# Zoe187419/ATE_replication_causalML

Hardware: AMD Instinct MI355X
Metric: rows/sec for DML-ATE cross-fit, N=1e7 p=500, 1/2/4/8 MI355X; ATE/SE parity (higher is better)
Workload: dtype bf16; 1 GPU; model=DML-PLR 5-fold cross-fit, CV-LASSO nuisances (100 lambdas, inner 4-fold CV), global_batch=10000000, seq_len=500, N=10000000, p=500, folds=5, parallelism=dp1, dgp=tutorial, n_kept=10000000, layout=blocked64+bytes8

## Files before the change

### ate_replication_causalml_amd/_native.py

```python
from __future__ import annotations

import ctypes
import os
from pathlib import Path

_LIBDIR = Path(__file__).resolve().parent / "_lib"
_hip = None
_cpu = None


class NativeMissing(RuntimeError):
    pass


class NativeError(RuntimeError):

    def __init__(self, name: str, status: int, detail: str):
        self.entry, self.status = name, status
        super().__init__(f"{name} failed with status {status}: {detail}")


HIP_ERRORS = {
    1: "hipErrorInvalidValue", 2: "hipErrorOutOfMemory", 3: "hipErrorNotInitialized",
    4: "hipErrorDeinitialized", 9: "hipErrorInvalidConfiguration",
    13: "hipErrorInvalidSymbol", 17: "hipErrorInvalidDevicePointer",
    21: "hipErrorInvalidMemcpyDirection", 35: "hipErrorInsufficientDriver",
    52: "hipErrorMissingConfiguration", 53: "hipErrorPriorLaunchFailure",
    98: "hipErrorInvalidDeviceFunction", 100: "hipErrorNoDevice", 101: "hipErrorInvalidDevice",
    200: "hipErrorInvalidImage", 201: "hipErrorInvalidContext", 209: "hipErrorNoBinaryForGpu",
    218: "hipErrorInvalidKernelFile", 400: "hipErrorInvalidHandle", 500: "hipErrorNotFound",
    600: "hipErrorNotReady", 700: "hipErrorIllegalAddress", 701: "hipErrorLaunchOutOfResources",
    702: "hipErrorLaunchTimeOut", 710: "hipErrorAssert", 719: "hipErrorLaunchFailure",
    720: "hipErrorCooperativeLaunchTooLarge", 801: "hipErrorNotSupported",
    900: "hipErrorStreamCaptureUnsupported", 901: "hipErrorStreamCaptureInvalidated",
    907: "hipErrorCapturedEvent", 999: "hipErrorUnknown",
}


def describe_status(rc: int) -> str:
    if rc < 0:
        return "rejected by the entry point's own argument check (no kernel launched)"
    return f"{HIP_ERRORS.get(rc, 'hipError?')} ({rc})"


c_void_p = ctypes.c_void_p
c_int = ctypes.c_int
c_int64 = ctypes.c_int64
c_uint64 = ctypes.c_uint64
c_double = ctypes.c_double

_SIGS = {
    "ate_gram_bf16": "pliipipipipppp",
    "ate_gram_bf16_pair": "pllipippipippippiip",
    "ate_gram_bf16_pair_bits": "pllipippipippippiip",
    "ate_last_error": "pi",
    "ate_last_stale_error": "pi",
    "ate_clear_errors": "",
    "ate_debug_bad_launch": "ip",
    "ate_check_kernel_resources": "pi",
    "ate_gram_f32": "plippipipippppp",
    "ate_gram_f64": "plippipipippppp",
    "ate_gram_tile_sizes": "pppp",
    "ate_chol_solve": "pipiipdpppppp",
    "ate_chol_solve_k": "pipipidppppp",
    "ate_spd_solve_batched": "ppiippp",
    "ate_predict": "ipllppiidipp",
    "ate_irls_update": "ipllppiiiiippppipp",
    "ate_irls_check": "piidippp",
    "ate_naive": "ippplpppp",
    "ate_clip_propensity": "pplpp",
    "ate_aipw": "ppppppldpppp",
    "ate_dml_moments": "ppplppp",
    "ate_dml_finalize": "pipp",
    "ate_boot_multinomial": "ppluiipp",
    "ate_boot_poisson": "ppluiilipp",
    "ate_enet_prepare": "piipipiipipipppppppp",
    "ate_enet_prepare_fused": "piipipiipipi" + "ppppppp" + "plp",
    "ate_enet_prepare_fused_clear": "piipipiipipi" + "ppppppp" + "pl" + "pl" + "p",
    "ate_enet_path": "pipiippppidddipppppippp",
    "ate_enet_coef": "ppiiiipppppppp",
    "ate_enet_cvloss_gauss": "pippiipppiiipp",
    "ate_cv_select": "pppiipippppip",
    "ate_enet_pick": "ppiiipppip",
    "ate_enet_cv_tail": "pippiipppi" + "pppppp" + "iiii" + "pppppppppppp",
    "ate_dml_resid_moments": "ipllpipipiiiiiippp",
    "ate_dml_resid_moments_final": "ipllpipipiiiiii" + "ppppp",
    "ate_dml_resid_exact": "pllpipipiiiiiiippp",
    "ate_dml_resid_terms": "ipllpipipiiiiii" + "ppp",
    "ate_cluster_chunk": "",
    "ate_cluster_work": "l",
    "ate_cluster_moments": "pplpplipppp",
    "ate_irm_score_moments": "ipllpipiipiiiiidippp",
    "ate_irm_score_moments_multi": "ipllpipiipipiiiiiidippp",
    "ate_irm_score_multi_smax": "",
    "ate_irm_scores": "ipllpipiipiiiiidipp",
    "ate_irm_sens_moments": "ipllpipiipiiiiidippp",
    "ate_irm_target_moments": "ipllpipiipiiiiidippp",
    "ate_irm_score_link": "ii" + "ipllpipiipiiiiidippp",
    "ate_iivm_moments": "ipllpipiipiiiiiiidippp",
    "ate_apo_moments": "ipllpipiipiiiiidippp",
    "ate_pliv_lds_max": "",
    "ate_pliv_moments": "ipllpipiippii" + "pppp",
    "ate_pliv_terms": "ipllpipiippii" + "pppp",
    "ate_group_boot": "pppliiuippp",
    "ate_group_boot_scratch": "iii",
    "ate_cate_moments": "ppplpiiippp",
    "ate_cate_moments_scratch": "iii",
    "ate_cate_boot": "ppplppiiiuippp",
    "ate_cate_boot_scratch": "iiii",
    "ate_rate_boot": "pppplliiuippp",
    "ate_rate_boot_scratch": "iii",
    "ate_policy_pair_hist": "ppppppliiipp",
    "ate_policy_pair_hist_scratch": "i",
    "ate_policy_search": "ppiilppp",
    "ate_lognet_path": "iplpiipipipdddippippppppppp",
    "ate_lognet_cvloss": "iplpiippipppipp",
    "ate_lognet_path_groups": "iplpiipipipppdpdiippppppppp",
    "ate_lognet_cvloss_set": "iplpiipipipppipp",
    "ate_dgp_fill": "iplllllp" + "uiipppp",
    "ate_dgp_pack_bits": "plpp",
    "ate_sel_block_rows": "",
    "ate_sel_gen_count": "upilllpp",
    "ate_sel_gen_flags": "upillpp",
    "ate_sel_gen_mark": "upiplllpiplp",
    "ate_forest_fit": "pppppi" + "pppppppp" + "ip",
    "ate_forest_predict": "ppiiipppppippip",
    "ate_forest_pack": "pippppppp",
    "ate_forest_scratch_bytes": "ii",
    "ate_forest_exact_scratch_bytes": "iiii",
    "ate_forest_fit_exact": "piiipppippppippppppppp",
    "ate_forest_predict16": "ppiiipppppppippip",
    "ate_bin_matrix": "plipppp",
    "ate_panel_xtv": "iplpipplipp",
    "ate_select_compact": "plppddpppp" + "p",
    "ate_gbdt_run": "ppp",
    "ate_lv_boot": "ppp",
    "ate_lv_classify": "pipiippp",
    "ate_lv_decide": "ppipipipippppp" + "iipip",
    "ate_lv_partition": "ppipippppipp",
    "ate_lv_scatter": "pppppippp",
    "ate_lv_children": "pippppp",
    "ate_lv_transpose": "piipip",
    "ate_gbdt_bin_panel": "pilpipppilpppl" + "p",
    "ate_gbdt_slab_entries": "liii",
    "ate_gbdt_slab2_entries": "li",
    "ate_gbdt_pair_root": "pppplllp",
    "ate_gbdt_apply": "plliipppp" + "p",
    "ate_panel_xv": "iplpipiplpp",
    "ate_col_moments": "pllipppp",
    "ate_standardize": "pllippp",
    "ate_interactions": "pllipl" + "p",
    "ate_scan_parts": "l",
    "ate_gbdt_limits": "p",
    "ate_excl_scan_i32": "plpppp",
    "ate_excl_scan_i64": "plpppp",
}
_RESTYPE = {"ate_forest_scratch_bytes": ctypes.c_int64,
            "ate_forest_exact_scratch_bytes": ctypes.c_int64, "ate_gbdt_slab_entries": ctypes.c_int64,
            "ate_gbdt_slab2_entries": ctypes.c_int64,
            "ate_scan_parts": ctypes.c_int64, "ate_group_boot_scratch": ctypes.c_int64,
            "ate_cate_moments_scratch": ctypes.c_int64,
            "ate_cate_boot_scratch": ctypes.c_int64,
            "ate_rate_boot_scratch": ctypes.c_int64,
            "ate_policy_pair_hist_scratch": ctypes.c_int64,
            "ate_cluster_work": ctypes.c_int64}
_CT = {"p": c_void_p, "i": c_int, "l": c_int64, "u": c_uint64, "d": c_double}

# ... 109 lines not shown
```

### ate_replication_causalml_amd/ops/enet.py

```python
from __future__ import annotations

import os
from dataclasses import dataclass

import numpy as np
import torch

from .. import _native
from ..reference import glmnet as ref
from .devconst import const, const_bytes


def _stream():
    return torch.cuda.current_stream().cuda_stream


CV_FUSED = os.environ.get("ATE_CV_FUSED", "1") not in ("", "0")


@dataclass
class EnetCvResult:
    lambdas: torch.Tensor
    nlam: torch.Tensor
    cvm: torch.Tensor
    cvsd: torch.Tensor
    sel: torch.Tensor
    coef_path: torch.Tensor
    coef_min: torch.Tensor
    coef_1se: torch.Tensor
    full_keys: list
    npass: torch.Tensor
    fold_npass: torch.Tensor | None = None
    fold_nlam: torch.Tensor | None = None
    spare_zero: torch.Tensor | None = None

    def check(self):
        bad = [] if self.fold_npass is None else \
            np.flatnonzero(self.fold_npass.cpu().numpy() < 0).tolist()
        if bad:
            from ..utils.guards import NumericalError
            raise NumericalError(f"CV fold path(s) {bad} timed out waiting for their "
                                 "full-data lambda sequence; selection is invalid")
        return self


def poison_if_truncated(fold_npass: torch.Tensor, *ts):
    bad = (fold_npass < 0).any()
    nan = torch.full((), float("nan"), dtype=torch.float64, device=fold_npass.device)
    return [torch.where(bad, nan, t) for t in ts]


def _zeroed(dev, *specs):
    sizes = [int(np.prod(sh)) * torch.empty((), dtype=dt).element_size() for sh, dt in specs]
    offs = np.concatenate([[0], np.cumsum([(b + 255) // 256 * 256 for b in sizes])])
    buf = torch.zeros(int(offs[-1]), dtype=torch.uint8, device=dev)
    return [buf[int(o):int(o) + b].view(dt).view(sh)
            for (sh, dt), o, b in zip(specs, offs[:-1], sizes)]


def _carved(dev, *specs):
    sizes = [int(np.prod(sh)) * torch.empty((), dtype=dt).element_size() for sh, dt in specs]
    offs = np.concatenate([[0], np.cumsum([(b + 255) // 256 * 256 for b in sizes])])
    buf = torch.empty(int(offs[-1]), dtype=torch.uint8, device=dev)
    return buf, [buf[int(o):int(o) + b].view(dt).view(sh)
                 for (sh, dt), o, b in zip(specs, offs[:-1], sizes)]


def _rescale_vp(vp, p):
    vp = np.ones(p) if vp is None else np.maximum(np.asarray(vp, float), 0)
    return vp * p / vp.sum()


def _cv_tables(nseg, full_sets, ycols, nreal, nlambda, full_y):
    ny = len(ycols)
    if full_sets is None:
        full_sets = [list(range(nseg))]
    tsets, tindex = [], {}

    def tid(segs):
        key = tuple(sorted(segs))
        if key not in tindex:
            tindex[key] = len(tsets)
            tsets.append(key)
        return tindex[key]

    full_t = [tid(fs) for fs in full_sets]
    fold_t, fold_hold = [], []
    for fs in full_sets:
        for s in fs:
            fold_t.append(tid([q for q in fs if q != s]))
            fold_hold.append(s)
    K = len(full_sets[0])
    assert all(len(fs) == K for fs in full_sets), "full sets must have equal fold counts"
    masks = np.zeros((len(tsets), nseg), dtype=np.uint8)
    for i, ts in enumerate(tsets):
        masks[i, list(ts)] = 1
    if full_y is None:
        ys_of = [list(range(ny))] * len(full_sets)
    else:
        if len(full_y) != len(full_sets) or any(not 0 <= int(y) < ny for y in full_y):
# ... 62 lines not shown


_PROB_DT = np.dtype([("train", "<i4"), ("y", "<i4"), ("src", "<i4"), ("nlam", "<i4")])


def _probs_tensor(probs, dev):
    return const_bytes(np.array(probs, dtype=_PROB_DT), dev)


def _cv_gpu(G, P, nseg, masks, xcols, ycols, p, ny, vp, one, full_probs, fold_probs, fold_ycol,
            fold_holds, fold_index, nfold, alpha, flmin, thresh, maxit, L, full_keys,
            panel_dtype):
    dev = G.device
    s = _stream()
    f64 = dict(dtype=torch.float64, device=dev)
    nt = masks.shape[0]
    masks_t = const(masks, torch.uint8, dev)
    xc = const(xcols, torch.int32, dev)
    yc = const(ycols, torch.int32, dev)
    c_f32 = int(panel_dtype != torch.float64)
    ldc = (p + 63) // 64 * 64
    nf = len(full_probs)
    probs_all = list(full_probs) + list(fold_probs)
    nq = len(probs_all)
    i32 = torch.int32
    c_dt = torch.float32 if c_f32 else torch.float64
    fused = CV_FUSED and L <= 256
    fused_prep = fused and nseg <= 8
    if fused:
        zspec = [((nq, L), torch.float64), ((nq,), i32), ((nq,), i32), ((nq,), i32), ((nf,), i32)]
        spare = zbuf = None
        if fused_prep:
            zbuf, (rsq, nlam, npass, progress, done, spare) = _carved(dev, *zspec, ((1,), i32))
            C = torch.empty((nt, p, ldc), dtype=c_dt, device=dev)
        else:
            zspec.append(((nt, p, ldc), c_dt))
            rsq, nlam, npass, progress, done, C = _zeroed(dev, *zspec)
        apath = torch.empty((nq, L, p), **f64)
    else:
        C, apath, rsq, nlam, npass, progress = _zeroed(
            dev, ((nt, p, ldc), c_dt), ((nq, L, p), torch.float64),
            ((nq, L), torch.float64), ((nq,), i32), ((nq,), i32), ((nq,), i32))
    g = torch.empty((nt, ny, p), **f64)
    xm = torch.empty((nt, p), **f64)
    xs = torch.empty((nt, p), **f64)
    ju = torch.empty((nt, p), dtype=torch.uint8, device=dev)
    ym = torch.empty((nt, ny), **f64)
    ys = torch.empty((nt, ny), **f64)
    nobs = torch.empty(nt, **f64)
    if fused_prep:
        lams = torch.empty((nq, L), **f64)
        _native.call("ate_enet_prepare_fused_clear", G.data_ptr(), nseg, P, masks_t.data_ptr(),
                     nt, xc.data_ptr(), p, one, yc.data_ptr(), ny, C.data_ptr(), c_f32,
                     g.data_ptr(), xm.data_ptr(), xs.data_ptr(), ju.data_ptr(), ym.data_ptr(),
                     ys.data_ptr(), nobs.data_ptr(), lams.data_ptr(), nq * L, zbuf.data_ptr(),
                     zbuf.numel() // 4, s)
    else:
        _native.call("ate_enet_prepare", G.data_ptr(), nseg, P, masks_t.data_ptr(), nt,
                     xc.data_ptr(), p, one, yc.data_ptr(), ny, C.data_ptr(), c_f32, g.data_ptr(),
                     xm.data_ptr(), xs.data_ptr(), ju.data_ptr(), ym.data_ptr(), ys.data_ptr(),
                     nobs.data_ptr(), s)
        lams = torch.full((nq, L), float("nan"), **f64)
    vp_t = const(np.asarray(vp, dtype=np.float64), torch.float64, dev)
    pr = _probs_tensor(probs_all, dev)
    lampub = torch.empty((nq, L), **f64)
    _native.call("ate_enet_path", C.data_ptr(), c_f32, g.data_ptr(), p, ny, ju.data_ptr(),
                 ys.data_ptr(), vp_t.data_ptr(), pr.data_ptr(), nq, alpha, flmin, thresh,
                 maxit, apath.data_ptr(), lams.data_ptr(), rsq.data_ptr(), nlam.data_ptr(),
                 npass.data_ptr(), L, progress.data_ptr(), lampub.data_ptr(), s)
    hold = const([0] * nf + list(fold_holds), torch.int32, dev)
    ycol_p = const([0] * nf + list(fold_ycol), torch.int32, dev)
    cvraw = torch.empty((nq, L), **f64)
    fidx = const(fold_index + nf, torch.int32, dev)
    nfold_t = const(nfold, torch.float64, dev)
    cvm = torch.empty((nf, L), **f64)
    cvsd = torch.empty((nf, L), **f64)
    sel = torch.empty((nf, 2), dtype=torch.int32, device=dev)
    K = fold_index.shape[1]
    cmin = torch.empty((nf, p + 1), **f64)
    c1se = torch.empty((nf, p + 1), **f64)
    fold_npass = npass[nf:]
    if fused:
        coef = torch.empty((nf, L, p + 1), **f64)
        _native.call("ate_enet_cv_tail", G.data_ptr(), P, hold.data_ptr(), xc.data_ptr(), p, one,
                     ycol_p.data_ptr(), apath.data_ptr(), pr.data_ptr(), ny, nlam.data_ptr(),
                     xm.data_ptr(), xs.data_ptr(), ju.data_ptr(), ym.data_ptr(), ys.data_ptr(), L,
                     nf, nq - nf, K, fidx.data_ptr(), nfold_t.data_ptr(), coef.data_ptr(),
                     cvraw.data_ptr(), cvm.data_ptr(), cvsd.data_ptr(), sel.data_ptr(),
                     cmin.data_ptr(), c1se.data_ptr(), fold_npass.data_ptr(), done.data_ptr(), s)
        return EnetCvResult(lams[:nf], nlam[:nf], cvm, cvsd, sel, coef, cmin, c1se, full_keys,
                            npass[:nf], fold_npass, nlam[nf:], spare)
    coef = torch.empty((nq, L, p + 1), **f64)
    _native.call("ate_enet_coef", apath.data_ptr(), pr.data_ptr(), nq, p, ny, L,
                 nlam.data_ptr(), xm.data_ptr(), xs.data_ptr(), ju.data_ptr(), ym.data_ptr(),
                 ys.data_ptr(), coef.data_ptr(), s)
    _native.call("ate_enet_cvloss_gauss", G.data_ptr(), P, hold.data_ptr(), xc.data_ptr(), p, one,
                 ycol_p.data_ptr(), coef.data_ptr(), nlam.data_ptr(), L, nf, nq - nf,
                 cvraw.data_ptr(), s)
    _native.call("ate_cv_select", cvraw.data_ptr(), fidx.data_ptr(), nfold_t.data_ptr(), K, nf,
                 nlam.data_ptr(), L, cvm.data_ptr(), cvsd.data_ptr(), sel.data_ptr(),
                 fold_npass.data_ptr(), nq - nf, s)
    _native.call("ate_enet_pick", coef.data_ptr(), sel.data_ptr(), p, L, nf, cmin.data_ptr(),
                 c1se.data_ptr(), fold_npass.data_ptr(), nq - nf, s)
    return EnetCvResult(lams[:nf], nlam[:nf], cvm, cvsd, sel, coef[:nf], cmin, c1se, full_keys,
                        npass[:nf], fold_npass, nlam[nf:])


def _cv_cpu(G, masks, xcols, ycols, p, ny, vp, one, full_probs, fold_probs, fold_ycol, fold_holds,
            fold_index, nfold, alpha, flmin, thresh, maxit, L, full_keys):
    Gn = G.double().cpu().numpy()
    nt = masks.shape[0]
    stats = []
    for t in range(nt):
        Gt = np.tensordot(masks[t].astype(float), Gn, axes=1)
        n = Gt[one, one]
        sx = Gt[one, xcols] / n
        vx = np.diag(Gt)[xcols] / n - sx * sx
        ju = vx > 0
        xs = np.where(ju, np.sqrt(np.maximum(vx, 0)), 1.0)
        Cm = (Gt[np.ix_(xcols, xcols)] / n - np.outer(sx, sx)) / np.outer(xs, xs)
        Cm[~ju, :] = 0
        Cm[:, ~ju] = 0
        Cm[np.flatnonzero(~ju), np.flatnonzero(~ju)] = 1.0
        gs, ymv, ysv = [], [], []
        for yc in ycols:
            my = Gt[one, yc] / n
            vy = Gt[yc, yc] / n - my * my
            sy = np.sqrt(vy) if vy > 0 else 1.0
            gj = np.where(ju, (Gt[xcols, yc] / n - sx * my) / (xs * sy), 0.0)
            gs.append(gj)
            ymv.append(my)
            ysv.append(sy)
        stats.append(dict(C=Cm, g=gs, xm=sx, xs=xs, ju=ju, ym=ymv, ys=ysv, n=n))

    def run(probs, src_paths):
        res = []
        for (t, y, src, nlam_req) in probs:
            st = stats[t]
            lam = None if src < 0 else src_paths[src].lambdas
            path = ref._elnet_core(st["C"], st["g"][y], np.ones(p), st["xm"], st["xs"], st["ym"][y],
                                   st["ys"][y], st["ju"], alpha, vp, lam, nlam_req or L, flmin,
                                   thresh, maxit)
            res.append(path)
        return res

    full = run(full_probs, None)
    folds = run(fold_probs, full)
    nf = len(full_probs)
    K = fold_index.shape[1]
    lams = np.full((nf, L), np.nan)
    nlam = np.zeros(nf, dtype=np.int32)
    coef = np.full((nf, L, p + 1), np.nan)
    for f, path in enumerate(full):
        m = len(path.lambdas)
        lams[f, :m] = path.lambdas
        nlam[f] = m
        coef[f, :m, 0] = path.a0
        coef[f, :m, 1:] = path.beta
    cvraw = np.full((len(fold_probs), L), np.nan)
    for q, path in enumerate(folds):
        Gh = Gn[fold_holds[q]]
        yc = fold_ycol[q]
        n = Gh[one, one]
        for m in range(len(path.lambdas)):
            a0, b = path.a0[m], path.beta[m]
            Gxx = Gh[np.ix_(xcols, xcols)]
            sse = (Gh[yc, yc] - 2 * a0 * Gh[one, yc] - 2 * b @ Gh[xcols, yc] + n * a0 * a0
                   + 2 * a0 * b @ Gh[xcols, one] + b @ Gxx @ b)
            cvraw[q, m] = sse / n
    cvm = np.full((nf, L), np.nan)
    cvsd = np.full((nf, L), np.nan)
    sel = np.zeros((nf, 2), dtype=np.int32)
    for f in range(nf):
        m = nlam[f]
        raw = cvraw[fold_index[f]][:, :m]
        cm, cs, i0, i1 = ref.cv_select(lams[f, :m], raw, nfold[f])
        cvm[f, :m], cvsd[f, :m] = cm, cs
        sel[f] = (i0, i1)
    cmin = np.stack([coef[f, sel[f, 0]] for f in range(nf)])
    c1se = np.stack([coef[f, sel[f, 1]] for f in range(nf)])
    t = torch.from_numpy
# ... 4 lines not shown
```

### csrc/enet.hip

```cpp
#include <cstdlib>

#include <utility>

#include "common.hpp"

#include <type_traits>

using namespace ate;

__device__ __forceinline__ double seg_sum(const double* __restrict__ G, int nseg, int P,
                                          const unsigned char* __restrict__ mk, int a, int b) {
  double acc = 0.0;
  for (int q = 0; q < nseg; ++q)
    if (mk[q]) acc += G[((int64_t)q * P + a) * P + b];
  return acc;
}

__device__ __forceinline__ void col_mean_var(double s1, double s2, double n, double& m,
                                             double& v) {
  m = s1 / n;
  v = s2 / n - m * m;
}
__device__ __forceinline__ double std_entry(double sab, double n, double ma, double mb,
                                            double sa, double sb) {
// ... 1553 lines not shown

ATE_API int ate_enet_path(const void* C, int c_f32, const void* g, int p, int ny, const void* ju,
                          const void* ys, const void* vp, const void* probs, int nprob,
                          double alpha, double flmin, double thr, int maxit, void* apath,
                          void* lams, void* rsqs, void* nlam_out, void* npass_out, int L,
                          void* progress, void* lampub, void* stream) {
  if (p > PMAX) return -2;
  if (nprob > 256) return -3;
  hipStream_t s = (hipStream_t)stream;
  const int nwg = (nprob + 7) / 8 * 8;
  const char* sm = getenv("ATE_ENET_SPIN_MAX");
  const long spin_max = sm ? atol(sm) : (1l << 26);
  const char* sp = getenv("ATE_ENET_S_PREFETCH");
  const int s_prefetch = sp ? atoi(sp) != 0 : 1;
#define LAUNCH_C(CTT, LS)                                                                      \
  ATE_LAUNCH((enet_path_kernel<CTT, LS>), dim3(nwg), dim3(NTH), 0, s, (const CTT*)C,   \
                     (const double*)g, p, ny, (const unsigned char*)ju, (const double*)ys,     \
                     (const double*)vp, (const EnetProblem*)probs, nprob, alpha, flmin, thr,   \
                     maxit, (double*)apath, (double*)lams, (double*)rsqs, (int*)nlam_out,     \
                     (int*)npass_out, L, (int*)progress, spin_max, (double*)lampub, s_prefetch)
  const bool lasso = alpha == 1.0;
  if (c_f32 && lasso) LAUNCH_C(float, true);
  else if (c_f32) LAUNCH_C(float, false);
  else if (lasso) LAUNCH_C(double, true);
  else LAUNCH_C(double, false);
#undef LAUNCH_C
  ATE_CHECK_LAUNCH();
  return 0;
}

template <class Store>
__device__ __forceinline__ double coef_row_terms(const double* __restrict__ a, int64_t tb, int p,
                                                 double ysq, const double* __restrict__ xm,
                                                 const double* __restrict__ xs,
                                                 const unsigned char* __restrict__ ju, int t0,
                                                 int stride, Store st) {
  double acc = 0.0;
  for (int j = t0; j < p; j += stride) {
    int64_t sj = tb + j;
    double b = ju[sj] ? a[j] * ysq / xs[sj] : 0.0;
    st(j, b);
    acc += b * xm[sj];
  }
  return acc;
}

__global__ void enet_coef_kernel(const double* __restrict__ apath, const EnetProblem* __restrict__ probs,
                                 int nprob, int p, int ny, int L, const int* __restrict__ nlam_out,
                                 const double* __restrict__ xm, const double* __restrict__ xs,
                                 const unsigned char* __restrict__ ju, const double* __restrict__ ym,
                                 const double* __restrict__ ys, double* __restrict__ coef) {
  const int q = blockIdx.y, m = blockIdx.x;
  if (q >= nprob || m >= L) return;
  const EnetProblem pr = probs[q];
  double* out = coef + ((int64_t)q * L + m) * (p + 1);
  if (m >= nlam_out[q]) {
    for (int j = threadIdx.x; j <= p; j += blockDim.x) out[j] = NAN;
    return;
  }
  const double* a = apath + ((int64_t)q * L + m) * p;
  const double ysq = ys[(int64_t)pr.train * ny + pr.y], ymq = ym[(int64_t)pr.train * ny + pr.y];
  __shared__ double smem[16];
  double acc[1] = {coef_row_terms(a, (int64_t)pr.train * p, p, ysq, xm, xs, ju, threadIdx.x,
                                  blockDim.x, [&](int j, double b) { out[1 + j] = b; })};
  block_sum<1>(acc, smem);
  if (threadIdx.x == 0) out[0] = ymq - acc[0];
}

ATE_API int ate_enet_coef(const void* apath, const void* probs, int nprob, int p, int ny, int L,
                          const void* nlam_out, const void* xm, const void* xs, const void* ju,
                          const void* ym, const void* ys, void* coef, void* stream) {
  ATE_LAUNCH(enet_coef_kernel, dim3(L, nprob), dim3(128), 0, (hipStream_t)stream,
                     (const double*)apath, (const EnetProblem*)probs, nprob, p, ny, L,
                     (const int*)nlam_out, (const double*)xm, (const double*)xs,
                     (const unsigned char*)ju, (const double*)ym, (const double*)ys,
                     (double*)coef);
  ATE_CHECK_LAUNCH();
  return 0;
}

constexpr int CVL = 8;
constexpr int CVK = PMAX / 64;

template <bool AGENT, class A0>
__device__ __forceinline__ void cvloss_chunk(
    const double* __restrict__ Gh, int P, const int* __restrict__ xcols, int p, int ones_col,
    int yc, double (*sbeta)[PMAX], int* sxc, unsigned char* snz, double (*sred)[3 * CVL], int nl,
    int m0, int L, double* __restrict__ cvq, A0 a0_of) {
  const int tid = threadIdx.x, lane = tid & 63, wid = tid >> 6;
  for (int j = tid; j < PMAX; j += 256) sxc[j] = j < p ? xcols[j] : xcols[0];
  __syncthreads();
  for (int j = tid; j < PMAX; j += 256) {
    bool any = false;
#pragma unroll
    for (int m = 0; m < CVL; ++m) any |= sbeta[m][j] != 0.0;
    snz[j] = any;
  }
  __syncthreads();
  double bl[CVK][CVL];
#pragma unroll
  for (int k = 0; k < CVK; ++k)
#pragma unroll
    for (int m = 0; m < CVL; ++m) bl[k][m] = sbeta[m][k * 64 + lane];
  int cl[CVK];
#pragma unroll
  for (int k = 0; k < CVK; ++k) cl[k] = sxc[k * 64 + lane];
  double quad[CVL], lin[CVL], sx[CVL];
#pragma unroll
  for (int m = 0; m < CVL; ++m) { quad[m] = 0.0; lin[m] = 0.0; sx[m] = 0.0; }
  if (wid == 0) {
#pragma unroll
    for (int k = 0; k < CVK; ++k) {
      if (k * 64 + lane >= p) continue;
      const double gy = Gh[(int64_t)cl[k] * P + yc], g1 = Gh[(int64_t)cl[k] * P + ones_col];
#pragma unroll
      for (int m = 0; m < CVL; ++m) {
        lin[m] = fma(bl[k][m], gy, lin[m]);
        sx[m] = fma(bl[k][m], g1, sx[m]);
      }
    }
  }
  auto next_row = [&](int a) {
    while (a < p && !snz[a]) a += 4;
    return a;
  };
  auto load_row = [&](int a, double* g) {
    const double* Gr = Gh + (int64_t)sxc[a] * P;
#pragma unroll
    for (int k = 0; k < CVK; ++k) g[k] = (k * 64 + lane < p) ? Gr[cl[k]] : 0.0;
  };
  double gn[CVK];
  int a = next_row(wid);
  if (a < p) load_row(a, gn);
  while (a < p) {
    double g[CVK];
#pragma unroll
    for (int k = 0; k < CVK; ++k) g[k] = gn[k];
    const int an = next_row(a + 4);
    if (an < p) load_row(an, gn);
#pragma unroll
    for (int m = 0; m < CVL; ++m) {
      double t = 0.0;
#pragma unroll
      for (int k = 0; k < CVK; ++k) t = fma(g[k], bl[k][m], t);
      quad[m] = fma(sbeta[m][a], t, quad[m]);
    }
    a = an;
  }
#pragma unroll
  for (int m = 0; m < CVL; ++m) {
    quad[m] = wave_sum(quad[m]);
    lin[m] = wave_sum(lin[m]);
    sx[m] = wave_sum(sx[m]);
  }
  if (lane == 0)
#pragma unroll
    for (int m = 0; m < CVL; ++m) {
      sred[wid][m] = quad[m];
      sred[wid][CVL + m] = lin[m];
      sred[wid][2 * CVL + m] = sx[m];
    }
  __syncthreads();
  if (tid < CVL && m0 + tid < L) {
    const int m = tid;
    if (m0 + m >= nl) {
      st_out<AGENT>(cvq + m0 + m, NAN);
    } else {
      const double qd = sred[0][m] + sred[1][m] + sred[2][m] + sred[3][m];
      const double ln = sred[0][CVL + m], s1 = sred[0][2 * CVL + m];
      const double a0 = a0_of(m);
      const double n = Gh[(int64_t)ones_col * P + ones_col];
      const double yy = Gh[(int64_t)yc * P + yc], sy = Gh[(int64_t)ones_col * P + yc];
      const double sse = yy - 2.0 * a0 * sy - 2.0 * ln + n * a0 * a0 + 2.0 * a0 * s1 + qd;
      st_out<AGENT>(cvq + m0 + m, sse / n);
    }
  }
}

__global__ __launch_bounds__(256) void enet_cvloss_gauss_kernel(
    const double* __restrict__ G, int P, const int* __restrict__ hold,
    const int* __restrict__ xcols, int p, int ones_col, const int* __restrict__ ycol_of_prob,
    const double* __restrict__ coef, const int* __restrict__ nlam_out, int L, int q0,
    double* __restrict__ cvraw) {
  const int q = q0 + blockIdx.x, m0 = (gridDim.y - 1 - blockIdx.y) * CVL;
  const int nl = nlam_out[q];
  const int tid = threadIdx.x, lane = tid & 63, wid = tid >> 6;
  if (m0 >= nl) {
    if (tid < CVL && m0 + tid < L) cvraw[(int64_t)q * L + m0 + tid] = NAN;
    return;
  }
  const double* Gh = G + (int64_t)hold[q] * P * P;
  const int yc = ycol_of_prob[q];
  __shared__ double sbeta[CVL][PMAX];
  __shared__ int sxc[PMAX];
  __shared__ unsigned char snz[PMAX];
  __shared__ double sred[4][3 * CVL];
  for (int e = tid; e < CVL * PMAX; e += 256) {
    const int m = e / PMAX, j = e % PMAX;
    const bool ok = j < p && m0 + m < nl;
    sbeta[m][j] = ok ? coef[((int64_t)q * L + m0 + m) * (p + 1) + 1 + j] : 0.0;
  }
  cvloss_chunk<false>(Gh, P, xcols, p, ones_col, yc, sbeta, sxc, snz, sred, nl, m0, L,
                      cvraw + (int64_t)q * L,
                      [&](int m) { return coef[((int64_t)q * L + m0 + m) * (p + 1)]; });
}

ATE_API int ate_enet_cvloss_gauss(const void* G, int P, const void* hold, const void* xcols, int p,
                                  int ones_col, const void* ycol_of_prob, const void* coef,
                                  const void* nlam_out, int L, int q0, int nprob, void* cvraw,
                                  void* stream) {
  if (p > PMAX) return -1;
  if (nprob <= 0) return 0;
  ATE_LAUNCH(enet_cvloss_gauss_kernel, dim3(nprob, (L + CVL - 1) / CVL), dim3(256), 0,
                     (hipStream_t)stream, (const double*)G, P, (const int*)hold,
                     (const int*)xcols, p, ones_col, (const int*)ycol_of_prob,
                     (const double*)coef, (const int*)nlam_out, L, q0, (double*)cvraw);
  ATE_CHECK_LAUNCH();
  return 0;
}

__device__ __forceinline__ bool any_truncated(const int* fnp, int nfp) {
  bool bad = false;
  if (fnp)
    for (int i = threadIdx.x; i < nfp; i += blockDim.x) bad |= fnp[i] < 0;
  return __syncthreads_or(bad) != 0;
}

__device__ __forceinline__ void cv_select_wave(
    const double* __restrict__ cvraw, const int* __restrict__ fold_probs,
    const double* __restrict__ nfold, int K, int f, const int* __restrict__ nlam_full, int L,
    double* __restrict__ cvm, double* __restrict__ cvsd, int* __restrict__ sel, bool bad,
    int lane, int& i_min, int& i_1se) {
  i_min = 0;
  i_1se = 0;
  if (bad) {
    for (int m = lane; m < L; m += 64) {
      cvm[(int64_t)f * L + m] = NAN;
      cvsd[(int64_t)f * L + m] = NAN;
    }
    if (lane == 0) { sel[2 * f] = 0; sel[2 * f + 1] = 0; }
    return;
  }
  const int nl = nlam_full[f];
  double wsum = 0.0;
  for (int k = 0; k < K; ++k) wsum += nfold[f * K + k];
  double mus[4], sds[4];
  double best = INFINITY;
  int imin = 0x7fffffff;
#pragma unroll
  for (int c = 0; c < 4; ++c) {
    const int m = c * 64 + lane;
    mus[c] = INFINITY;
    sds[c] = 0.0;
    if (m >= nl) {
      if (m < L) {
        cvm[(int64_t)f * L + m] = NAN;
        cvsd[(int64_t)f * L + m] = NAN;
      }
      continue;
    }
    double mu = 0.0;
    for (int k = 0; k < K; ++k) mu += nfold[f * K + k] * cvraw[(int64_t)fold_probs[f * K + k] * L + m];
    mu /= wsum;
    double var = 0.0;
    for (int k = 0; k < K; ++k) {
      double d = cvraw[(int64_t)fold_probs[f * K + k] * L + m] - mu;
      var += nfold[f * K + k] * d * d;
    }
    const double sd = sqrt(var / wsum / (double)(K - 1));
    cvm[(int64_t)f * L + m] = mu;
    cvsd[(int64_t)f * L + m] = sd;
    mus[c] = mu;
    sds[c] = sd;
    if (mu < best) { best = mu; imin = m; }
  }
#pragma unroll
  for (int o = 32; o > 0; o >>= 1) {
    const double ob = __shfl_xor(best, o, 64);
    const int oi = __shfl_xor(imin, o, 64);
    if (ob < best || (ob == best && oi < imin)) { best = ob; imin = oi; }
  }
  if (imin == 0x7fffffff) imin = 0;
  const int oc = imin >> 6, ol = imin & 63;
  double mine = 0.0;
#pragma unroll
  for (int c = 0; c < 4; ++c)
    if (c == oc) mine = mus[c] + sds[c];
  const double thr1 = __shfl(mine, ol, 64);
  int i1 = imin;
#pragma unroll
  for (int c = 0; c < 4; ++c) {
    const uint64_t b = __ballot(c * 64 + lane < nl && mus[c] <= thr1);
    if (b) { i1 = c * 64 + __ffsll((unsigned long long)b) - 1; break; }
  }
  if (lane == 0) {
    sel[2 * f] = imin;
    sel[2 * f + 1] = i1;
  }
  i_min = imin;
  i_1se = i1;
}

__global__ __launch_bounds__(64) void cv_select_kernel(
    const double* __restrict__ cvraw, const int* __restrict__ fold_probs,
    const double* __restrict__ nfold, int K, int nfull, const int* __restrict__ nlam_full, int L,
    double* __restrict__ cvm, double* __restrict__ cvsd, int* __restrict__ sel,
    const int* __restrict__ fnp, int nfp) {
  const int f = blockIdx.x;
  const int lane = threadIdx.x;
  if (f >= nfull) return;
  int i0, i1;
  cv_select_wave(cvraw, fold_probs, nfold, K, f, nlam_full, L, cvm, cvsd, sel,
                 any_truncated(fnp, nfp), lane, i0, i1);
}

ATE_API int ate_cv_select(const void* cvraw, const void* fold_probs, const void* nfold, int K,
                          int nfull, const void* nlam_full, int L, void* cvm, void* cvsd, void* sel,
                          const void* fold_npass, int nfp, void* stream) {
  if (L > 256) return -1;
  ATE_LAUNCH(cv_select_kernel, dim3(nfull), dim3(64), 0, (hipStream_t)stream,
                     (const double*)cvraw, (const int*)fold_probs, (const double*)nfold, K, nfull,
                     (const int*)nlam_full, L, (double*)cvm, (double*)cvsd, (int*)sel,
                     (const int*)fold_npass, nfp);
  ATE_CHECK_LAUNCH();
  return 0;
}

__global__ void enet_pick_kernel(const double* __restrict__ coef, const int* __restrict__ sel,
                                 int p, int L, int nfull, double* __restrict__ out_min,
                                 double* __restrict__ out_1se, const int* __restrict__ fnp,
                                 int nfp) {
  const int f = blockIdx.x, which = blockIdx.y;
  double* out = which ? out_1se : out_min;
  const bool bad = any_truncated(fnp, nfp);
  const int m = sel[2 * f + which];
  for (int j = threadIdx.x; j <= p; j += blockDim.x)
    out[(int64_t)f * (p + 1) + j] = bad ? NAN : coef[((int64_t)f * L + m) * (p + 1) + j];
}

ATE_API int ate_enet_pick(const void* coef, const void* sel, int p, int L, int nfull,
                          void* out_min, void* out_1se, const void* fold_npass, int nfp,
                          void* stream) {
  ATE_LAUNCH(enet_pick_kernel, dim3(nfull, 2), dim3(128), 0, (hipStream_t)stream,
                     (const double*)coef, (const int*)sel, p, L, nfull, (double*)out_min,
                     (double*)out_1se, (const int*)fold_npass, nfp);
  ATE_CHECK_LAUNCH();
  return 0;
}

__global__ __launch_bounds__(256) void enet_cv_tail_kernel(
    const double* __restrict__ G, int P, const int* __restrict__ hold,
    const int* __restrict__ xcols, int p, int ones_col, const int* __restrict__ ycol_of_prob,
    const double* __restrict__ apath, const EnetProblem* __restrict__ probs, int ny,
    const int* __restrict__ nlam_out, const double* __restrict__ xm,
    const double* __restrict__ xs, const unsigned char* __restrict__ ju,
    const double* __restrict__ ym, const double* __restrict__ ys, int L, int nf, int nfp, int K,
    const int* __restrict__ fold_probs, const double* __restrict__ nfold, double* coef,
    double* cvraw, double* cvm, double* cvsd, int* sel, double* out_min, double* out_1se,
    const int* __restrict__ fnp, int* done) {
  const int tid = threadIdx.x, lane = tid & 63, wid = tid >> 6;
  const int nch = (L + CVL - 1) / CVL, ncv = nfp * nch;
  const int b = blockIdx.x;
  __shared__ double sbeta[CVL][PMAX];
  __shared__ int sxc[PMAX];
  __shared__ unsigned char snz[PMAX];
  __shared__ double sred[4][3 * CVL];
  __shared__ double sw[CVL][2], sa0[CVL];
  __shared__ int slast, ssel[2];
  int f;
  if (b < ncv) {
    const int q = nf + b % nfp, m0 = (nch - 1 - b / nfp) * CVL;
    const EnetProblem pr = probs[q];
    f = pr.ulam_src;
    ATE_DASSERT(f >= 0 && f < nf && pr.train >= 0 && pr.y >= 0 && pr.y < ny);
    const int nl = nlam_out[q];
    if (m0 >= nl) {
      if (tid < CVL && m0 + tid < L) st_out<true>(cvraw + (int64_t)q * L + m0 + tid, NAN);
    } else {
      const double* Gh = G + (int64_t)hold[q] * P * P;
      const int yc = ycol_of_prob[q];
      const double ysq = ys[(int64_t)pr.train * ny + pr.y], ymq = ym[(int64_t)pr.train * ny + pr.y];
      for (int e = tid; e < CVL * PMAX; e += 256) (&sbeta[0][0])[e] = 0.0;
      __syncthreads();
      const int half = tid >> 7, t = tid & 127;
#pragma unroll
      for (int r = 0; r < CVL / 2; ++r) {
        const int m = 2 * r + half;
        double acc = 0.0;
        if (m0 + m < nl)
          acc = coef_row_terms(apath + ((int64_t)q * L + m0 + m) * p, (int64_t)pr.train * p, p,
                               ysq, xm, xs, ju, t, 128,
                               [&](int j, double bj) { sbeta[m][j] = bj; });
        acc = wave_sum(acc);
        if (lane == 0) sw[m][wid & 1] = acc;
      }
      __syncthreads();
      if (tid < CVL) {
        double s = 0.0;
        for (int w = 0; w < 2; ++w) s += sw[tid][w];
        sa0[tid] = ymq - s;
      }
      cvloss_chunk<true>(Gh, P, xcols, p, ones_col, yc, sbeta, sxc, snz, sred, nl, m0, L,
                         cvraw + (int64_t)q * L, [&](int m) { return sa0[m]; });
    }
  } else {
    f = (b - ncv) / L;
    const int m = (b - ncv) % L;
    ATE_DASSERT(f < nf);
    const EnetProblem pr = probs[f];
    double* out = coef + ((int64_t)f * L + m) * (p + 1);
    if (m >= nlam_out[f]) {
      for (int j = tid; j <= p; j += 256) st_out<true>(out + j, NAN);
    } else {
      const double ysq = ys[(int64_t)pr.train * ny + pr.y], ymq = ym[(int64_t)pr.train * ny + pr.y];
      double acc = 0.0;
      if (tid < 128)
        acc = coef_row_terms(apath + ((int64_t)f * L + m) * p, (int64_t)pr.train * p, p, ysq, xm,
                             xs, ju, tid, 128,
                             [&](int j, double bj) { st_out<true>(out + 1 + j, bj); });
      acc = wave_sum(acc);
      if (lane == 0 && wid < 2) sw[0][wid] = acc;
      __syncthreads();
      if (tid == 0) {
        double s = 0.0;
        for (int w = 0; w < 2; ++w) s += sw[0][w];
        st_out<true>(out, ymq - s);
      }
    }
  }
  wait_stores();
  __syncthreads();
  if (tid == 0) {
    const int total = L + K * nch;
    const int old = __hip_atomic_fetch_add(done + f, 1, __ATOMIC_RELAXED, __HIP_MEMORY_SCOPE_AGENT);
    ATE_DASSERT(old >= 0 && old < total);
    slast = old == total - 1;
  }
  __syncthreads();
  if (!slast) return;
  __builtin_amdgcn_fence(__ATOMIC_ACQUIRE, "agent");
  const bool bad = any_truncated(fnp, nfp);
  if (wid == 0) {
    int i0, i1;
    cv_select_wave(cvraw, fold_probs, nfold, K, f, nlam_out, L, cvm, cvsd, sel, bad, lane, i0, i1);
    if (lane == 0) { ssel[0] = i0; ssel[1] = i1; }
  }
  __syncthreads();
  for (int which = 0; which < 2; ++which) {
    double* out = which ? out_1se : out_min;
    const int m = ssel[which];
    ATE_DASSERT(m >= 0 && m < L);
    for (int j = tid; j <= p; j += 256)
      out[(int64_t)f * (p + 1) + j] = bad ? NAN : coef[((int64_t)f * L + m) * (p + 1) + j];
  }
}

ATE_API int ate_enet_cv_tail(const void* G, int P, const void* hold, const void* xcols, int p,
                             int ones_col, const void* ycol_of_prob, const void* apath,
                             const void* probs, int ny, const void* nlam_out, const void* xm,
                             const void* xs, const void* ju, const void* ym, const void* ys, int L,
                             int nf, int nfp, int K, const void* fold_probs, const void* nfold,
                             void* coef, void* cvraw, void* cvm, void* cvsd, void* sel,
                             void* out_min, void* out_1se, const void* fold_npass, void* done,
                             void* stream) {
  if (p > PMAX || p < 1 || L > 256 || L < 1) return -1;
  if (nf < 1 || K < 1 || nfp != nf * K) return -1;
  const int nch = (L + CVL - 1) / CVL;
  ATE_LAUNCH(enet_cv_tail_kernel, dim3(nfp * nch + nf * L), dim3(256), 0, (hipStream_t)stream,
             (const double*)G, P, (const int*)hold, (const int*)xcols, p, ones_col,
             (const int*)ycol_of_prob, (const double*)apath, (const EnetProblem*)probs, ny,
             (const int*)nlam_out, (const double*)xm, (const double*)xs,
             (const unsigned char*)ju, (const double*)ym, (const double*)ys, L, nf, nfp, K,
             (const int*)fold_probs, (const double*)nfold, (double*)coef, (double*)cvraw,
             (double*)cvm, (double*)cvsd, (int*)sel, (double*)out_min, (double*)out_1se,
             (const int*)fold_npass, (int*)done);
  ATE_CHECK_LAUNCH();
  return 0;
}
```

Measured before the change: 2.453 billion rows/s.

## Add configurable multi-row prefetch depth to CV-loss Gram row loop

Result: no change. 2.460 billion rows/s (median of 2 runs) (+0.3%).

```diff
diff --git a/ate_replication_causalml_amd/_native.py b/ate_replication_causalml_amd/_native.py
--- a/ate_replication_causalml_amd/_native.py
+++ b/ate_replication_causalml_amd/_native.py
@@ -80,9 +80,11 @@
     "ate_enet_path": "pipiippppidddipppppippp",
     "ate_enet_coef": "ppiiiipppppppp",
     "ate_enet_cvloss_gauss": "pippiipppiiipp",
+    "ate_enet_cvloss_gauss_d": "pippiipppiiipip",
     "ate_cv_select": "pppiipippppip",
     "ate_enet_pick": "ppiiipppip",
     "ate_enet_cv_tail": "pippiipppi" + "pppppp" + "iiii" + "pppppppppppp",
+    "ate_enet_cv_tail_d": "pippiipppi" + "pppppp" + "iiii" + "ppppppppppp" + "ip",
     "ate_dml_resid_moments": "ipllpipipiiiiiippp",
     "ate_dml_resid_moments_final": "ipllpipipiiiiii" + "ppppp",
     "ate_dml_resid_exact": "pllpipipiiiiiiippp",
diff --git a/ate_replication_causalml_amd/ops/enet.py b/ate_replication_causalml_amd/ops/enet.py
--- a/ate_replication_causalml_amd/ops/enet.py
+++ b/ate_replication_causalml_amd/ops/enet.py
@@ -16,6 +16,10 @@
 
 
 CV_FUSED = os.environ.get("ATE_CV_FUSED", "1") not in ("", "0")
+
+CVL_DEPTH = int(os.environ.get("ATE_CVL_DEPTH", "1"))
+if not 1 <= CVL_DEPTH <= 4:
+    raise ValueError(f"ATE_CVL_DEPTH must be 1, 2, 3 or 4, not {CVL_DEPTH}")
 
 
 @dataclass
@@ -244,21 +248,22 @@
     fold_npass = npass[nf:]
     if fused:
         coef = torch.empty((nf, L, p + 1), **f64)
-        _native.call("ate_enet_cv_tail", G.data_ptr(), P, hold.data_ptr(), xc.data_ptr(), p, one,
+        _native.call("ate_enet_cv_tail_d", G.data_ptr(), P, hold.data_ptr(), xc.data_ptr(), p, one,
                      ycol_p.data_ptr(), apath.data_ptr(), pr.data_ptr(), ny, nlam.data_ptr(),
                      xm.data_ptr(), xs.data_ptr(), ju.data_ptr(), ym.data_ptr(), ys.data_ptr(), L,
                      nf, nq - nf, K, fidx.data_ptr(), nfold_t.data_ptr(), coef.data_ptr(),
                      cvraw.data_ptr(), cvm.data_ptr(), cvsd.data_ptr(), sel.data_ptr(),
-                     cmin.data_ptr(), c1se.data_ptr(), fold_npass.data_ptr(), done.data_ptr(), s)
+                     cmin.data_ptr(), c1se.data_ptr(), fold_npass.data_ptr(), done.data_ptr(),
+                     CVL_DEPTH, s)
         return EnetCvResult(lams[:nf], nlam[:nf], cvm, cvsd, sel, coef, cmin, c1se, full_keys,
                             npass[:nf], fold_npass, nlam[nf:], spare)
     coef = torch.empty((nq, L, p + 1), **f64)
     _native.call("ate_enet_coef", apath.data_ptr(), pr.data_ptr(), nq, p, ny, L,
                  nlam.data_ptr(), xm.data_ptr(), xs.data_ptr(), ju.data_ptr(), ym.data_ptr(),
                  ys.data_ptr(), coef.data_ptr(), s)
-    _native.call("ate_enet_cvloss_gauss", G.data_ptr(), P, hold.data_ptr(), xc.data_ptr(), p, one,
-                 ycol_p.data_ptr(), coef.data_ptr(), nlam.data_ptr(), L, nf, nq - nf,
-                 cvraw.data_ptr(), s)
+    _native.call("ate_enet_cvloss_gauss_d", G.data_ptr(), P, hold.data_ptr(), xc.data_ptr(), p,
+                 one, ycol_p.data_ptr(), coef.data_ptr(), nlam.data_ptr(), L, nf, nq - nf,
+                 cvraw.data_ptr(), CVL_DEPTH, s)
     _native.call("ate_cv_select", cvraw.data_ptr(), fidx.data_ptr(), nfold_t.data_ptr(), K, nf,
                  nlam.data_ptr(), L, cvm.data_ptr(), cvsd.data_ptr(), sel.data_ptr(),
                  fold_npass.data_ptr(), nq - nf, s)
diff --git a/csrc/enet.hip b/csrc/enet.hip
--- a/csrc/enet.hip
+++ b/csrc/enet.hip
@@ -1659,12 +1659,30 @@
 constexpr int CVL = 8;
 constexpr int CVK = PMAX / 64;
 
-template <bool AGENT, class A0>
+#ifdef ENET_PROF
+constexpr int CVT_N = 20, CVT_WG = 4096;
+__device__ unsigned long long cv_tail_prof[CVT_WG][CVT_N];
+#define CVT_SET(k, v) do { if (blockIdx.x < CVT_WG) cv_tail_prof[blockIdx.x][k] = (unsigned long long)(v); } while (0)
+#define CVT_ROW() ++cvt_rows_
+#else
+#define CVT_SET(k, v) do { } while (0)
+#define CVT_ROW() do { } while (0)
+#endif
+
+constexpr int CVL_DEPTH = 1;
+constexpr int vmcnt_only(int n) { return (n & 0xF) | ((n >> 4) << 14) | 0x0F70; }
+
+template <int D, bool AGENT, class A0>
 __device__ __forceinline__ void cvloss_chunk(
     const double* __restrict__ Gh, int P, const int* __restrict__ xcols, int p, int ones_col,
     int yc, double (*sbeta)[PMAX], int* sxc, unsigned char* snz, double (*sred)[3 * CVL], int nl,
     int m0, int L, double* __restrict__ cvq, A0 a0_of) {
+  static_assert(D >= 1 && 8 * (D - 1) < 64, "the counted wait must fit vmcnt");
   const int tid = threadIdx.x, lane = tid & 63, wid = tid >> 6;
+#ifdef ENET_PROF
+  int cvt_rows_ = 0;
+  if (AGENT && tid == 0) { CVT_SET(6, wall_clock64()); CVT_SET(7, D); }
+#endif
   for (int j = tid; j < PMAX; j += 256) sxc[j] = j < p ? xcols[j] : xcols[0];
   __syncthreads();
   for (int j = tid; j < PMAX; j += 256) {
@@ -1682,10 +1700,10 @@
   int cl[CVK];
 #pragma unroll
   for (int k = 0; k < CVK; ++k) cl[k] = sxc[k * 64 + lane];
-  double quad[CVL], lin[CVL], sx[CVL];
-#pragma unroll
-  for (int m = 0; m < CVL; ++m) { quad[m] = 0.0; lin[m] = 0.0; sx[m] = 0.0; }
   if (wid == 0) {
+    double lin[CVL], sx[CVL];
+#pragma unroll
+    for (int m = 0; m < CVL; ++m) { lin[m] = 0.0; sx[m] = 0.0; }
 #pragma unroll
     for (int k = 0; k < CVK; ++k) {
       if (k * 64 + lane >= p) continue;
@@ -1696,25 +1714,26 @@
         sx[m] = fma(bl[k][m], g1, sx[m]);
       }
     }
-  }
-  auto next_row = [&](int a) {
-    while (a < p && !snz[a]) a += 4;
-    return a;
-  };
-  auto load_row = [&](int a, double* g) {
-    const double* Gr = Gh + (int64_t)sxc[a] * P;
-#pragma unroll
-    for (int k = 0; k < CVK; ++k) g[k] = (k * 64 + lane < p) ? Gr[cl[k]] : 0.0;
-  };
-  double gn[CVK];
-  int a = next_row(wid);
-  if (a < p) load_row(a, gn);
-  while (a < p) {
-    double g[CVK];
-#pragma unroll
-    for (int k = 0; k < CVK; ++k) g[k] = gn[k];
-    const int an = next_row(a + 4);
-    if (an < p) load_row(an, gn);
+#pragma unroll
+    for (int m = 0; m < CVL; ++m) {
+      lin[m] = wave_sum(lin[m]);
+      sx[m] = wave_sum(sx[m]);
+    }
+    if (lane == 0)
+#pragma unroll
+      for (int m = 0; m < CVL; ++m) {
+        sred[0][CVL + m] = lin[m];
+        sred[0][2 * CVL + m] = sx[m];
+      }
+  }
+  double quad[CVL];
+#pragma unroll
+  for (int m = 0; m < CVL; ++m) quad[m] = 0.0;
+#ifdef ENET_PROF
+  if (AGENT && lane == 0) CVT_SET(12 + wid, wall_clock64());
+#endif
+  auto apply_row = [&](int a, const double* g) {
+    CVT_ROW();
 #pragma unroll
     for (int m = 0; m < CVL; ++m) {
       double t = 0.0;
@@ -1722,21 +1741,79 @@
       for (int k = 0; k < CVK; ++k) t = fma(g[k], bl[k][m], t);
       quad[m] = fma(sbeta[m][a], t, quad[m]);
     }
-    a = an;
-  }
-#pragma unroll
-  for (int m = 0; m < CVL; ++m) {
-    quad[m] = wave_sum(quad[m]);
-    lin[m] = wave_sum(lin[m]);
-    sx[m] = wave_sum(sx[m]);
-  }
+  };
+  if constexpr (D == 1) {
+    auto next_row = [&](int a) {
+      while (a < p && !snz[a]) a += 4;
+      return a;
+    };
+    auto load_row = [&](int a, double* g) {
+      const double* Gr = Gh + (int64_t)sxc[a] * P;
+#pragma unroll
+      for (int k = 0; k < CVK; ++k) g[k] = (k * 64 + lane < p) ? Gr[cl[k]] : 0.0;
+    };
+    double gn[CVK];
+    int a = next_row(wid);
+    if (a < p) load_row(a, gn);
+    while (a < p) {
+      double g[CVK];
+#pragma unroll
+      for (int k = 0; k < CVK; ++k) g[k] = gn[k];
+      const int an = next_row(a + 4);
+      if (an < p) load_row(an, gn);
+      apply_row(a, g);
+      a = an;
+    }
+  } else {
+    auto next_row = [&](int a) {
+      while (a < p && !__builtin_amdgcn_readfirstlane((int)snz[a])) a += 4;
+      return a;
+    };
+    unsigned cb[CVK];
+#pragma unroll
+    for (int k = 0; k < CVK; ++k) cb[k] = (unsigned)cl[k] * 8u;
+    auto issue_row = [&](int a, double* g) {
+      const int col = __builtin_amdgcn_readfirstlane(sxc[a < p ? a : 0]);
+      const char* Gr = (const char*)(Gh + (int64_t)col * P);
+#pragma unroll
+      for (int k = 0; k < CVK; ++k) {
+        unsigned off = cb[k];
+        asm volatile("" : "+v"(off));
+        g[k] = *(const double*)(Gr + off);
+      }
+    };
+    double g[D][CVK];
+    int ar[D];
+    int nxt = next_row(__builtin_amdgcn_readfirstlane(wid));
+#pragma unroll
+    for (int s = 0; s < D; ++s) {
+      ar[s] = nxt;
+      issue_row(nxt, g[s]);
+      nxt = next_row(nxt + 4);
+    }
+    while (ar[0] < p) {
+#pragma unroll
+      for (int s = 0; s < D; ++s) {
+        if (ar[s] < p) {
+          __builtin_amdgcn_s_waitcnt(vmcnt_only(8 * (D - 1)));
+          apply_row(ar[s], g[s]);
+        }
+#pragma unroll
+        for (int m = 0; m < CVL; ++m) asm volatile("" : "+v"(quad[m]));
+        ar[s] = nxt;
+        issue_row(nxt, g[s]);
+        nxt = next_row(nxt + 4);
+      }
+    }
+  }
+#ifdef ENET_PROF
+  if (AGENT && lane == 0) { CVT_SET(16 + wid, wall_clock64()); CVT_SET(8 + wid, cvt_rows_); }
+#endif
+#pragma unroll
+  for (int m = 0; m < CVL; ++m) quad[m] = wave_sum(quad[m]);
   if (lane == 0)
 #pragma unroll
-    for (int m = 0; m < CVL; ++m) {
-      sred[wid][m] = quad[m];
-      sred[wid][CVL + m] = lin[m];
-      sred[wid][2 * CVL + m] = sx[m];
-    }
+    for (int m = 0; m < CVL; ++m) sred[wid][m] = quad[m];
   __syncthreads();
   if (tid < CVL && m0 + tid < L) {
     const int m = tid;
@@ -1754,7 +1831,8 @@
   }
 }
 
-__global__ __launch_bounds__(256) void enet_cvloss_gauss_kernel(
+template <int D>
+__global__ __launch_bounds__(256, 2) void enet_cvloss_gauss_kernel(
     const double* __restrict__ G, int P, const int* __restrict__ hold,
     const int* __restrict__ xcols, int p, int ones_col, const int* __restrict__ ycol_of_prob,
     const double* __restrict__ coef, const int* __restrict__ nlam_out, int L, int q0,
@@ -1777,23 +1855,37 @@
     const bool ok = j < p && m0 + m < nl;
     sbeta[m][j] = ok ? coef[((int64_t)q * L + m0 + m) * (p + 1) + 1 + j] : 0.0;
   }
-  cvloss_chunk<false>(Gh, P, xcols, p, ones_col, yc, sbeta, sxc, snz, sred, nl, m0, L,
+  cvloss_chunk<D, false>(Gh, P, xcols, p, ones_col, yc, sbeta, sxc, snz, sred, nl, m0, L,
                       cvraw + (int64_t)q * L,
                       [&](int m) { return coef[((int64_t)q * L + m0 + m) * (p + 1)]; });
+}
+
+ATE_API int ate_enet_cvloss_gauss_d(const void* G, int P, const void* hold, const void* xcols,
+                                    int p, int ones_col, const void* ycol_of_prob,
+                                    const void* coef, const void* nlam_out, int L, int q0,
+                                    int nprob, void* cvraw, int depth, void* stream) {
+  if (p > PMAX || depth < 1 || depth > 4) return -1;
+  if (nprob <= 0) return 0;
+#define LAUNCH_D(DD)                                                                           \
+  ATE_LAUNCH((enet_cvloss_gauss_kernel<DD>), dim3(nprob, (L + CVL - 1) / CVL), dim3(256), 0,   \
+             (hipStream_t)stream, (const double*)G, P, (const int*)hold, (const int*)xcols, p, \
+             ones_col, (const int*)ycol_of_prob, (const double*)coef, (const int*)nlam_out, L, \
+             q0, (double*)cvraw)
+  if (depth == 1) LAUNCH_D(1);
+  else if (depth == 2) LAUNCH_D(2);
+  else if (depth == 3) LAUNCH_D(3);
+  else LAUNCH_D(4);
+#undef LAUNCH_D
+  ATE_CHECK_LAUNCH();
+  return 0;
 }
 
 ATE_API int ate_enet_cvloss_gauss(const void* G, int P, const void* hold, const void* xcols, int p,
                                   int ones_col, const void* ycol_of_prob, const void* coef,
                                   const void* nlam_out, int L, int q0, int nprob, void* cvraw,
                                   void* stream) {
-  if (p > PMAX) return -1;
-  if (nprob <= 0) return 0;
-  ATE_LAUNCH(enet_cvloss_gauss_kernel, dim3(nprob, (L + CVL - 1) / CVL), dim3(256), 0,
-                     (hipStream_t)stream, (const double*)G, P, (const int*)hold,
-                     (const int*)xcols, p, ones_col, (const int*)ycol_of_prob,
-                     (const double*)coef, (const int*)nlam_out, L, q0, (double*)cvraw);
-  ATE_CHECK_LAUNCH();
-  return 0;
+  return ate_enet_cvloss_gauss_d(G, P, hold, xcols, p, ones_col, ycol_of_prob, coef, nlam_out, L,
+                                 q0, nprob, cvraw, CVL_DEPTH, stream);
 }
 
 __device__ __forceinline__ bool any_truncated(const int* fnp, int nfp) {
@@ -1925,7 +2017,8 @@
   return 0;
 }
 
-__global__ __launch_bounds__(256) void enet_cv_tail_kernel(
+template <int D>
+__global__ __launch_bounds__(256, 2) void enet_cv_tail_kernel(
     const double* __restrict__ G, int P, const int* __restrict__ hold,
     const int* __restrict__ xcols, int p, int ones_col, const int* __restrict__ ycol_of_prob,
     const double* __restrict__ apath, const EnetProblem* __restrict__ probs, int ny,
@@ -1938,6 +2031,15 @@
   const int tid = threadIdx.x, lane = tid & 63, wid = tid >> 6;
   const int nch = (L + CVL - 1) / CVL, ncv = nfp * nch;
   const int b = blockIdx.x;
+#ifdef ENET_PROF
+  if (tid == 0) {
+    unsigned xcc;
+    asm volatile("s_getreg_b32 %0, hwreg(HW_REG_XCC_ID, 0, 4)" : "=s"(xcc));
+    for (int k = 0; k < CVT_N; ++k) CVT_SET(k, 0);
+    CVT_SET(0, wall_clock64());
+    CVT_SET(2, xcc);
+  }
+#endif
   __shared__ double sbeta[CVL][PMAX];
   __shared__ int sxc[PMAX];
   __shared__ unsigned char snz[PMAX];
@@ -1947,6 +2049,9 @@
   int f;
   if (b < ncv) {
     const int q = nf + b % nfp, m0 = (nch - 1 - b / nfp) * CVL;
+#ifdef ENET_PROF
+    if (tid == 0) { CVT_SET(3, m0 >= nlam_out[q] ? 2 : 1); CVT_SET(4, q); CVT_SET(5, m0); }
+#endif
     const EnetProblem pr = probs[q];
     f = pr.ulam_src;
     ATE_DASSERT(f >= 0 && f < nf && pr.train >= 0 && pr.y >= 0 && pr.y < ny);
@@ -1977,13 +2082,16 @@
         for (int w = 0; w < 2; ++w) s += sw[tid][w];
         sa0[tid] = ymq - s;
       }
-      cvloss_chunk<true>(Gh, P, xcols, p, ones_col, yc, sbeta, sxc, snz, sred, nl, m0, L,
+      cvloss_chunk<D, true>(Gh, P, xcols, p, ones_col, yc, sbeta, sxc, snz, sred, nl, m0, L,
                          cvraw + (int64_t)q * L, [&](int m) { return sa0[m]; });
     }
   } else {
     f = (b - ncv) / L;
     const int m = (b - ncv) % L;
     ATE_DASSERT(f < nf);
+#ifdef ENET_PROF
+    if (tid == 0) { CVT_SET(3, 3); CVT_SET(4, f); CVT_SET(5, m); }
+#endif
     const EnetProblem pr = probs[f];
     double* out = coef + ((int64_t)f * L + m) * (p + 1);
     if (m >= nlam_out[f]) {
@@ -2005,6 +2113,10 @@
       }
     }
   }
+#ifdef ENET_PROF
+  __syncthreads();
+  if (tid == 0) CVT_SET(1, wall_clock64());
+#endif
   wait_stores();
   __syncthreads();
   if (tid == 0) {
@@ -2032,6 +2144,35 @@
   }
 }
 
+ATE_API int ate_enet_cv_tail_d(const void* G, int P, const void* hold, const void* xcols, int p,
+                               int ones_col, const void* ycol_of_prob, const void* apath,
+                               const void* probs, int ny, const void* nlam_out, const void* xm,
+                               const void* xs, const void* ju, const void* ym, const void* ys,
+                               int L, int nf, int nfp, int K, const void* fold_probs,
+                               const void* nfold, void* coef, void* cvraw, void* cvm, void* cvsd,
+                               void* sel, void* out_min, void* out_1se, const void* fold_npass,
+                               void* done, int depth, void* stream) {
+  if (p > PMAX || p < 1 || L > 256 || L < 1) return -1;
+  if (nf < 1 || K < 1 || nfp != nf * K || depth < 1 || depth > 4) return -1;
+  const int nch = (L + CVL - 1) / CVL;
+#define LAUNCH_D(DD)                                                                           \
+  ATE_LAUNCH((enet_cv_tail_kernel<DD>), dim3(nfp * nch + nf * L), dim3(256), 0,                \
+             (hipStream_t)stream, (const double*)G, P, (const int*)hold, (const int*)xcols, p, \
+             ones_col, (const int*)ycol_of_prob, (const double*)apath,                         \
+             (const EnetProblem*)probs, ny, (const int*)nlam_out, (const double*)xm,           \
+             (const double*)xs, (const unsigned char*)ju, (const double*)ym,                   \
+             (const double*)ys, L, nf, nfp, K, (const int*)fold_probs, (const double*)nfold,   \
+             (double*)coef, (double*)cvraw, (double*)cvm, (double*)cvsd, (int*)sel,            \
+             (double*)out_min, (double*)out_1se, (const int*)fold_npass, (int*)done)
+  if (depth == 1) LAUNCH_D(1);
+  else if (depth == 2) LAUNCH_D(2);
+  else if (depth == 3) LAUNCH_D(3);
+  else LAUNCH_D(4);
+#undef LAUNCH_D
+  ATE_CHECK_LAUNCH();
+  return 0;
+}
+
 ATE_API int ate_enet_cv_tail(const void* G, int P, const void* hold, const void* xcols, int p,
                              int ones_col, const void* ycol_of_prob, const void* apath,
                              const void* probs, int ny, const void* nlam_out, const void* xm,
@@ -2040,17 +2181,14 @@
                              void* coef, void* cvraw, void* cvm, void* cvsd, void* sel,
                              void* out_min, void* out_1se, const void* fold_npass, void* done,
                              void* stream) {
-  if (p > PMAX || p < 1 || L > 256 || L < 1) return -1;
-  if (nf < 1 || K < 1 || nfp != nf * K) return -1;
-  const int nch = (L + CVL - 1) / CVL;
-  ATE_LAUNCH(enet_cv_tail_kernel, dim3(nfp * nch + nf * L), dim3(256), 0, (hipStream_t)stream,
-             (const double*)G, P, (const int*)hold, (const int*)xcols, p, ones_col,
-             (const int*)ycol_of_prob, (const double*)apath, (const EnetProblem*)probs, ny,
-             (const int*)nlam_out, (const double*)xm, (const double*)xs,
-             (const unsigned char*)ju, (const double*)ym, (const double*)ys, L, nf, nfp, K,
-             (const int*)fold_probs, (const double*)nfold, (double*)coef, (double*)cvraw,
-             (double*)cvm, (double*)cvsd, (int*)sel, (double*)out_min, (double*)out_1se,
-             (const int*)fold_npass, (int*)done);
-  ATE_CHECK_LAUNCH();
-  return 0;
-}
+  return ate_enet_cv_tail_d(G, P, hold, xcols, p, ones_col, ycol_of_prob, apath, probs, ny,
+                            nlam_out, xm, xs, ju, ym, ys, L, nf, nfp, K, fold_probs, nfold, coef,
+                            cvraw, cvm, cvsd, sel, out_min, out_1se, fold_npass, done, CVL_DEPTH,
+                            stream);
+}
+
+#ifdef ENET_PROF
+extern "C" __attribute__((visibility("default"))) int ate_cv_tail_prof_read(void* host) {
+  return (int)hipMemcpyFromSymbol(host, HIP_SYMBOL(cv_tail_prof), sizeof(cv_tail_prof));
+}
+#endif
```
